# statgen/demuxlet

Measured on AMD Instinct MI355X. Metric: cell-SNP-sample triples/sec (singlet+doublet llk); HBM GB/s vs roofline, higher is better.
Workload: dtype f64

## Files before the change

demuxlet_amd/csrc/dmx_engine.hip:

```cpp
#include <hip/hip_runtime.h>

#include <algorithm>
#include <chrono>
#include <cmath>
#include <mutex>
#include <cstdlib>
#include <cstring>
#include <condition_variable>
#include <deque>
#include <new>
#include <memory>
#include <functional>
#include <thread>
#include <type_traits>
#include <unordered_map>
#include <cxxabi.h>
#include <string>
#include <numeric>
#include <vector>

#include "dmx_internal.hpp"
extern char** environ;
#include "dmx_log.hpp"
#include "dmx_engine_state.hpp"
// ... 2803 lines not shown
  const int64_t np = cell_ok ? pv.cell_pair_off[cell + 1] - p_beg : 0;
  int64_t rd_base = cell_ok ? pv.cell_read_off[cell] : 0;

  const int KB = (V + NK - 1) / NK;
  const int JS = TPC / KB;
  const int jl = tid / KB, kb = tid % KB;
  const int j = (int)blockIdx.y * JS + jl;
  const bool owner = jl < JS && j < V;
  double acc[NK][A];
#pragma unroll
  for (int kk = 0; kk < NK; ++kk) { acc[kk][0] = 0.0; acc[kk][1] = 0.0; }
  bool ok = true;
  const DmxLogPins lk = dmx_log_pins();
  int uj[2] = {0, 0}, uk[2] = {0, 0};
  if constexpr (SYMU) {
#pragma unroll
    for (int su = 0; su < 2; ++su) { const int u = tid + TPC * su; uj[su] = u & (kUV - 1); uk[su] = (uj[su] + 1 + (u >> kUSh)) & (kUV - 1); }
  }
  const int ti1 = tid >> 1, n1 = tid & 1;
  double acc00 = 0.0;
  const int row_len = V * 3;

  for (int64_t tbase = 0; tbase < np; tbase += TP) {
    const int tp = (int)min((int64_t)TP, np - tbase);
    if (tid < TP) {
      const bool v = tid < tp;
      const uint32_t n = v ? load_nrd(pv.pair_nrd, p_beg + tbase + tid, nrd_width) : 0u;
      const uint32_t incl = seg_scan_incl<TP>(n);
      s_cnt[tid] = n;
      s_off[tid] = rd_base + (int64_t)(incl - n);
      s_snp[tid] = v ? (pv.pair_snp ? pv.pair_snp[p_beg + tbase + tid] : (int32_t)(tbase + tid)) : 0;
    }
    DMX_K2_SYNC();
    rd_base = s_off[tp - 1] + (int64_t)s_cnt[tp - 1];
    {
      int r = tid % row_len, ti = tid / row_len;
      const int dr = TPC % row_len, dt = TPC / row_len;
      while (ti < tp) {
        s_g[ti * GS + r] = (g_t)g[(size_t)s_snp[ti] * row_len + r];
        r += dr; ti += dt;
        if (r >= row_len) { r -= row_len; ++ti; }
      }
    }
    if (tid < 2 * TP) {
      const bool on = ti1 < tp;
      const uint32_t cnt = on ? s_cnt[ti1] : 0u;
      const int64_t off = on ? s_off[ti1] : 0;
      const uint32_t rd4 = load_rd4(pv, off, cnt);
      double vf[9];
      const int32_t fi = pfin ? certify_final_index(cnt, rd4) : -1;
      if (!__any(fi < 0)) {
        const double* fp = pfin + (size_t)fi * kCFinStride + (n1 ? 0 : 5);
        const double f0 = fp[0], f1 = fp[1], f2 = fp[2], f3 = n1 ? fp[3] : 0.0, f4 = n1 ? fp[4] : 0.0;
        const double f5[5] = {f0, f1, f2, f3, f4};
#pragma unroll
        for (int l = 0; l < 3; ++l)
#pragma unroll
          for (int m = 0; m < 3; ++m) vf[l * 3 + m] = n1 ? f5[l + m] : f5[l];
      } else if (pseed) {
        double q5[5], wA5[5], wR5[5];
#pragma unroll
        for (int q = 0; q < 5; ++q) {
          const int l = n1 ? (q > 2 ? 2 : q) : min(q, 2), m = n1 ? q - l : 0;
          const double p = 0.5 * l + (m - l) * 0.5 * (n1 ? 0.5 : 0.0);
          wA5[q] = p;
          wR5[q] = 1.0 - p;
        }
        certify_pair_values<5, false>(pv, cnt, off, rd4, s_tab, wA5, wR5, n1, q5, pseed);
#pragma unroll
        for (int l = 0; l < 3; ++l)
#pragma unroll
          for (int m = 0; m < 3; ++m) vf[l * 3 + m] = n1 ? q5[l + m] : q5[l];
      } else {
      double pG[9], wA[9], wR[9];
#pragma unroll
      for (int i = 0; i < 9; ++i) { pG[i] = 1.0; wA[i] = s_w[n1][i]; wR[i] = s_w[n1][9 + i]; }
      for (uint32_t r = 0; __any(r < cnt); ++r) {
        const bool live = r < cnt;
        const uint32_t byte = live ? (r < 4 ? (rd4 >> (8 * r)) & 0xFFu : (uint32_t)pv.reads[off + r]) : 0u;
        const uint32_t bq = byte & 127u;
        const bool alt = (byte >> 7) != 0;
        const double pR = alt ? s_tab[128 + bq] : s_tab[bq];
        const double pA = alt ? s_tab[bq] : s_tab[128 + bq];
        double mx = 0.0;
        if (live) {
#pragma unroll
          for (int i = 0; i < 9; ++i) {
            pG[i] *= (pR * wR[i] + pA * wA[i]);
            mx = fmax(mx, pG[i]);
          }
        }
        {
          const double o = shfl_xor1(mx);
          mx = fmax(mx, o);
        }
        if (live) {
          if (cnt <= kSafeReads) {
            const double y = rcp_refined(mx);
#pragma unroll
            for (int i = 0; i < 9; ++i) pG[i] = div_by(pG[i], mx, y);
          } else {
#pragma unroll
            for (int i = 0; i < 9; ++i) pG[i] /= mx;
          }
        }
      }
      double mx = 0.0;
#pragma unroll
      for (int i = 0; i < 9; ++i) {
        pG[i] += 1e-6;
        mx = fmax(mx, pG[i]);
      }
      {
        const double o = shfl_xor1(mx);
        mx = fmax(mx, o);
      }
      {
        const double y = rcp_refined(mx);
#pragma unroll
        for (int i = 0; i < 9; ++i) vf[i] = div_by(pG[i], mx, y);
      }
      }
      if (on) {
        const double* g0 = gp0 + (size_t)s_snp[ti1] * 3;
        const double q0 = g0[0], q1 = g0[1], q2 = g0[2];
        const double qq[3] = {q0, q1, q2};
        double sum = 0.0;
#pragma unroll
        for (int l = 0; l < 3; ++l)
#pragma unroll
          for (int m = 0; m < 3; ++m) {
            const double v = vf[l * 3 + m];
            s_pG[(ti1 * 2 + n1) * 9 + l * 3 + m] = v;
            sum += ((qq[l] * qq[m]) * v);
          }
        ok &= __builtin_amdgcn_class(sum, 0x100);
        s_t00[n1 * T00 + ti1] = dmx_log2_fast(sum, s_log);
      }
    }
    DMX_K2_SYNC();
    if (tid < 2) {
      const double* row = &s_t00[tid * T00];
      if (tp == TP) {
        double2 v[TP / 2];
#pragma unroll
        for (int i = 0; i < TP / 2; ++i) v[i] = *reinterpret_cast<const double2*>(&row[2 * i]);
#pragma unroll
        for (int i = 0; i < TP / 2; ++i) { acc00 += v[i].x; acc00 += v[i].y; }
      } else {
        for (int i = 0; i < tp; ++i) acc00 += row[i];
      }
    }
    if constexpr (SYMU) {
      for (int ti = 0; ti < tp; ++ti) {
        const double* P = &s_pG[ti * 18];
        const double Q[3] = {P[0], P[3], P[6]};
        const double P1[5] = {P[9], P[10], P[11], P[14], P[17]};
        const g_t* gr = &s_g[ti * GS];
#pragma unroll
        for (int su = 0; su < 2; ++su) {
          const int js = uj[su], ks = uk[su];
          const double a[3] = {(double)gr[js * 3], (double)gr[js * 3 + 1], (double)gr[js * 3 + 2]};
          const double b[3] = {(double)gr[ks * 3], (double)gr[ks * 3 + 1], (double)gr[ks * 3 + 2]};
          double E[3][3];
#pragma unroll
          for (int l = 0; l < 3; ++l)
#pragma unroll
            for (int m = 0; m < 3; ++m) E[l][m] = a[l] * b[m];
          {
            double s_jk0 = E[0][0] * Q[0], s_kj0 = E[0][0] * Q[0];
#pragma unroll
            for (int l = 0; l < 3; ++l)
#pragma unroll
              for (int m = 0; m < 3; ++m) {
                if (l == 0 && m == 0) continue;
                s_jk0 += (E[l][m] * Q[l]);
                s_kj0 += (E[m][l] * Q[l]);
              }
            acc[2 * su][0] += dmx_log2_fast_pinned(s_jk0, s_log, lk);
            acc[2 * su + 1][0] += dmx_log2_fast_pinned(s_kj0, s_log, lk);
          }
          {
#pragma unroll
            for (int l = 0; l < 3; ++l)
#pragma unroll
              for (int m = 0; m < 3; ++m) E[l][m] = E[l][m] * P1[l + m];
            double s_jk1 = E[0][0], s_kj1 = E[0][0];
#pragma unroll
            for (int l = 0; l < 3; ++l)
#pragma unroll
              for (int m = 0; m < 3; ++m) {
                if (l == 0 && m == 0) continue;
                s_jk1 += E[l][m];
                s_kj1 += E[m][l];
              }
            acc[2 * su][1] += dmx_log2_fast_pinned(s_jk1, s_log, lk);
            acc[2 * su + 1][1] += dmx_log2_fast_pinned(s_kj1, s_log, lk);
          }
        }
      }
    } else
    if (owner) {
      for (int ti = 0; ti < tp; ++ti) {
        const double* P = &s_pG[ti * 18];
        double P0[9], P1[9];
#pragma unroll
        for (int i = 0; i < 9; ++i) { P0[i] = P[i]; P1[i] = P[9 + i]; }
        const g_t* gr = &s_g[ti * GS];
        const double a0 = (double)gr[j * 3], a1 = (double)gr[j * 3 + 1], a2 = (double)gr[j * 3 + 2];
        const double aj[3] = {a0, a1, a2};
#pragma unroll
        for (int kk = 0; kk < NK; ++kk) {
          const int k = min(kb * NK + kk, V - 1);
          const double b0 = (double)gr[k * 3], b1 = (double)gr[k * 3 + 1], b2 = (double)gr[k * 3 + 2];
          const double bk[3] = {b0, b1, b2};
          double s0 = (aj[0] * bk[0]) * P0[0], s1 = (aj[0] * bk[0]) * P1[0];
#pragma unroll
          for (int l = 0; l < 3; ++l)
#pragma unroll
            for (int m = 0; m < 3; ++m) {
              if (l == 0 && m == 0) continue;
              const double gp = aj[l] * bk[m];
              s0 += (gp * P0[l * 3 + m]);
              s1 += (gp * P1[l * 3 + m]);
            }
          if (CHK) ok &= __builtin_amdgcn_class(s0, 0x100) && __builtin_amdgcn_class(s1, 0x100);
          acc[kk][0] += dmx_log2_fast_pinned(s0, s_log, lk);
          acc[kk][1] += dmx_log2_fast_pinned(s1, s_log, lk);
        }
      }
    }
    DMX_K2_SYNC();
  }
  if (cell_ok) {
    if constexpr (SYMU) {
#pragma unroll
      for (int su = 0; su < 2; ++su) {
        const int u = tid + TPC * su, d = 1 + (u >> kUSh);
        if (d < kUV / 2 || (d == kUV / 2 && uj[su] < kUV / 2)) {
          double* o = grid + (((size_t)cell * V + uj[su]) * V + uk[su]) * A;
          o[0] = acc[2 * su][0]; o[1] = acc[2 * su][1];
          double* o2 = grid + (((size_t)cell * V + uk[su]) * V + uj[su]) * A;
          o2[0] = acc[2 * su + 1][0]; o2[1] = acc[2 * su + 1][1];
        }
      }
    } else
    if (owner) {
#pragma unroll
      for (int kk = 0; kk < NK; ++kk) {
        const int k = kb * NK + kk;
        if (k < V) {
          double* o = grid + (((size_t)cell * V + j) * V + k) * A;
          o[0] = acc[kk][0]; o[1] = acc[kk][1];
        }
      }
    }
    if (tid < 2 && blockIdx.y == 0) l00[(size_t)cell * A + tid] = acc00;
    if (!ok) flag_cell(flagged, cell);
  }
#undef DMX_K2_SYNC
}
template <int TPC, int NK, int MINW = 1, bool GD = false, bool CHK = true, int TP = 32>
__global__ __launch_bounds__(kThreads, (MINW == 1 && TPC == 64) ? 3 : MINW) void k_doublet_a2(PileupView pv, int nrd_width, const float* __restrict__ g,
                                                         const double* __restrict__ gp0, const double* __restrict__ tabs,
                                                         const double* __restrict__ alpha,
                                                         const int32_t* __restrict__ sched, int32_t V, int32_t GS,
                                                         double* __restrict__ grid, double* __restrict__ l00,
                                                         uint8_t* __restrict__ flagged, const double* __restrict__ pfin, const double* __restrict__ pseed) {
  a2_body<TPC, NK, MINW, GD, CHK, TP, false>(pv, nrd_width, g, gp0, tabs, alpha, sched, V, GS, grid, l00, flagged, pfin, pseed);
}
template <int MINW>
__global__ __launch_bounds__(kThreads, MINW) void k_doublet_a2u(PileupView pv, int nrd_width, const float* __restrict__ g,
                                                          const double* __restrict__ gp0, const double* __restrict__ tabs,
                                                          const double* __restrict__ alpha,
                                                          const int32_t* __restrict__ sched, int32_t V, int32_t GS,
                                                          double* __restrict__ grid, double* __restrict__ l00,
                                                          uint8_t* __restrict__ flagged, const double* __restrict__ pfin, const double* __restrict__ pseed) {
  a2_body<256, 4, MINW, true, false, 32, true>(pv, nrd_width, g, gp0, tabs, alpha, sched, V, GS, grid, l00, flagged, pfin, pseed);
}
__global__ __launch_bounds__(kThreads, 3) void k_doublet_a2u16(PileupView pv, int nrd_width, const float* __restrict__ g,
                                                          const double* __restrict__ gp0, const double* __restrict__ tabs,
                                                          const double* __restrict__ alpha,
                                                          const int32_t* __restrict__ sched, int32_t V, int32_t GS,
                                                          double* __restrict__ grid, double* __restrict__ l00,
                                                          uint8_t* __restrict__ flagged, const double* __restrict__ pfin, const double* __restrict__ pseed) {
  a2_body<64, 4, 1, false, false, 32, true>(pv, nrd_width, g, gp0, tabs, alpha, sched, V, GS, grid, l00, flagged, pfin, pseed);
}

template <int TPC, int NK>
__global__ __launch_bounds__(kThreads, 3) void k_doublet_a2f(PileupView pv, int nrd_width, const float* __restrict__ g,
                                                         const double* __restrict__ gp0, const double* __restrict__ tabs,
                                                         const double* __restrict__ alpha,
                                                         const int32_t* __restrict__ sched, int32_t V, int32_t GS,
                                                         double* __restrict__ grid, double* __restrict__ l00,
                                                         uint8_t* __restrict__ flagged) {
  constexpr int A = 2, TP = 32;
  constexpr int CPW = kThreads / TPC;
  constexpr int T00 = TP + 2;
#define DMX_K2_SYNC() do { if (TPC == 64) { DMX_WAVE_LDS_ORDER(); } else { __syncthreads(); } } while (0)
  extern __shared__ __attribute__((aligned(16))) unsigned char s_raw[];
  __shared__ double s_tab[kTab2];
  const double* s_log = s_tab + kLut2;
  const int t = threadIdx.x;
  stage_k2_tables(s_tab, tabs, t, kThreads);
  __syncthreads();

  const int cw = t / TPC, tid = t % TPC;
  constexpr bool SHARE = TPC > 64;
  constexpr int SUB = 8;
  const int VU = V;
  const size_t cell_bytes = (size_t)TP * 18 * 8 + (size_t)TP * GS * 4 + 2 * T00 * 8 + TP * (4 + 4 + 8) + (SHARE ? (size_t)SUB * 2 * VU * 32 : 0);
  unsigned char* base = s_raw + (size_t)cw * cell_bytes;
  double* s_pG = (double*)base;
  float* s_g = (float*)(base + (size_t)TP * 18 * 8);
  double* s_t00 = (double*)((unsigned char*)s_g + (size_t)TP * GS * 4);
  int64_t* s_off = (int64_t*)(s_t00 + 2 * T00);
  int32_t* s_snp = (int32_t*)(s_off + TP);
  uint32_t* s_cnt = (uint32_t*)(s_snp + TP);
  double* s_u = (double*)(s_cnt + TP);

  const int slot = blockIdx.x * CPW + cw;
  if (TPC == 64 && slot >= pv.B) return;
  const bool cell_ok = slot < pv.B;
  const int32_t cell = cell_ok ? sched[slot] : 0;
  const int64_t p_beg = cell_ok ? pv.cell_pair_off[cell] : 0;
  const int64_t np = cell_ok ? pv.cell_pair_off[cell + 1] - p_beg : 0;
  int64_t rd_base = cell_ok ? pv.cell_read_off[cell] : 0;

  const int KB = (V + NK - 1) / NK;
  const int JS = TPC / KB;
  const int jl = tid / KB, kb = tid % KB;
  const int j = (int)blockIdx.y * JS + jl;
  const bool owner = jl < JS && j < V;
  double acc[NK][A];
#pragma unroll
  for (int kk = 0; kk < NK; ++kk) { acc[kk][0] = 0.0; acc[kk][1] = 0.0; }
  bool ok = true;
  const DmxLogPins lk = dmx_log_pins();
  const int ti1 = tid >> 1, n1 = tid & 1;
  double wA[9], wR[9];
  {
    const double al = alpha[n1];
#pragma unroll
    for (int l = 0; l < 3; ++l)
#pragma unroll
      for (int m = 0; m < 3; ++m) {
        const double p = 0.5 * l + (m - l) * 0.5 * al;
        wA[l * 3 + m] = p;
        wR[l * 3 + m] = 1.0 - p;
      }
  }
  double acc00 = 0.0;
  const int row_len = V * 3;
// ... 782 lines not shown
            for (int l = 0; l < 3; ++l)
#pragma unroll
              for (int m = 0; m < 3; ++m) {
                if (l == 0 && m == 0) continue;
                s_jk0 += (E[l][m] * Q[l]);
                s_kj0 += (E[m][l] * Q[l]);
              }
            acc[i][0] += dmx_log2_fast_pinned(s_jk0, s_log, lk);
            acc[i][2] += dmx_log2_fast_pinned(s_kj0, s_log, lk);
          }
          if (!ROOMY) __builtin_amdgcn_sched_barrier(0);
          {
            const double P[5] = {ROOMY ? Pr[0] : lds_read_f64(&pq[0]), ROOMY ? Pr[1] : lds_read_f64(&pq[1]), ROOMY ? Pr[2] : lds_read_f64(&pq[2]),
                                 ROOMY ? Pr[3] : lds_read_f64(&pq[3]), ROOMY ? Pr[4] : lds_read_f64(&pq[4])};
#pragma unroll
            for (int l = 0; l < 3; ++l)
#pragma unroll
              for (int m = 0; m < 3; ++m) E[l][m] = E[l][m] * P[l + m];
            double s_jk1 = E[0][0], s_kj1 = E[0][0];
#pragma unroll
            for (int l = 0; l < 3; ++l)
#pragma unroll
              for (int m = 0; m < 3; ++m) {
                if (l == 0 && m == 0) continue;
                s_jk1 += E[l][m];
                s_kj1 += E[m][l];
              }
            acc[i][1] += dmx_log2_fast_pinned(s_jk1, s_log, lk);
            acc[i][3] += dmx_log2_fast_pinned(s_kj1, s_log, lk);
          }
          __builtin_amdgcn_sched_barrier(0);
        }
        if (slab == 0) {
          double sd = 0.0;
#pragma unroll
          for (int l = 0; l < 3; ++l)
#pragma unroll
            for (int m = 0; m < 3; ++m) {
              const double v = pq[5 + l + dg[m]];
              const double term = (a[l] * a[m]) * v;
              sd = (l == 0 && m == 0) ? term : sd + term;
            }
          accd += dmx_log2_fast_pinned(sd, s_log, lk);
        }
      }
      DMX_WAVE_LDS_ORDER();
    }
  }
  double* G = grid + (size_t)cell * V * V * A;
#pragma unroll
  for (int i = 0; i < (DIAG_ONLY ? 0 : NU); ++i) {
    const int d = 1 + 2 * (NU * slab + i) + h, k = kk[i];
    if (d < 16 || j < 16) {
      G[((size_t)j * V + k) * A] = acc[i][0]; G[((size_t)j * V + k) * A + 1] = acc[i][1];
      G[((size_t)k * V + j) * A] = acc[i][2]; G[((size_t)k * V + j) * A + 1] = acc[i][3];
    }
  }
  if (slab == 0) {
    G[((size_t)j * V + j) * A + h] = accd;
    if (!DIAG_ONLY && tid < 2) l00[(size_t)cell * A + tid] = acc00;
  }
}

template <int MINW, int VP = 32>
__global__ __launch_bounds__(kThreads, MINW) void k_doublet_diag(PileupView pv, int nrd_width, const float* __restrict__ g,
                                                           const double* __restrict__ tabs, const int32_t* __restrict__ sched,
                                                           double* __restrict__ grid, const double* __restrict__ pfin, const double* __restrict__ pseed) {
  static_assert(VP == 32 || VP == 16, "panel");
  constexpr int V = VP, A = 2, TPC = VP, TP = VP / 2, CPW = kThreads / TPC, row_len = 3 * V, PB = 8, WPC = 64 / TPC;
  __shared__ double s_tab[kTab2];
  __shared__ double s_w[2][10];
  __shared__ __attribute__((aligned(16))) double s_pq_all[CPW][TP][8];
  __shared__ int64_t s_off_all[CPW][TP];
  __shared__ int32_t s_snp_all[CPW][TP];
  __shared__ uint32_t s_cnt_all[CPW][TP];
  const double* s_log = s_tab + kLut2;
  const int t = threadIdx.x;
  stage_k2_tables(s_tab, tabs, t, kThreads);
  if (t < 10) {
    const int n = t / 5, q = t % 5;
    const int l = n ? (q > 2 ? 2 : q) : min(q, 2), m = n ? q - l : 0;
    const double p = 0.5 * l + (m - l) * 0.5 * (n ? 0.5 : 0.0);
    s_w[n][q] = p;
    s_w[n][5 + q] = 1.0 - p;
  }
  __syncthreads();
  const int cw = t / TPC, tid = t % TPC;
  double* s_pq = &s_pq_all[cw][0][0];
  int64_t* s_off = s_off_all[cw]; int32_t* s_snp = s_snp_all[cw]; uint32_t* s_cnt = s_cnt_all[cw];
  const int slot = blockIdx.x * CPW + cw;
  if ((blockIdx.x * CPW + (cw & ~(WPC - 1))) >= pv.B) return;
  const bool cell_ok = slot < pv.B;
  const int32_t cell = cell_ok ? sched[slot] : 0;
  const int64_t p_beg = cell_ok ? pv.cell_pair_off[cell] : 0;
  const int64_t np = cell_ok ? pv.cell_pair_off[cell + 1] - p_beg : 0;
  int64_t rd_base = cell_ok ? pv.cell_read_off[cell] : 0;
  int64_t np_w = np;
#pragma unroll
  for (int d = TPC; d < 64; d <<= 1) { const int64_t o = __shfl_xor(np_w, d); np_w = np_w > o ? np_w : o; }
  const int j = tid;
  double acc0 = 0.0, acc1 = 0.0;
  const DmxLogPins lk = dmx_log_pins();
  const int ti1 = tid >> 1, n1 = tid & 1;
  for (int64_t tbase = 0; tbase < np_w; tbase += TP) {
    const int tp = (int)max((int64_t)0, min((int64_t)TP, np - tbase));
    if (tid < TP) {
      const bool v = tid < tp;
      const uint32_t n = v ? load_nrd(pv.pair_nrd, p_beg + tbase + tid, nrd_width) : 0u;
      const int32_t sn = v ? (pv.pair_snp ? pv.pair_snp[p_beg + tbase + tid] : (int32_t)(tbase + tid)) : 0;
      const uint32_t incl = seg_scan_incl<TP>(n);
      s_cnt[tid] = n;
      s_off[tid] = rd_base + (int64_t)(incl - n);
      s_snp[tid] = sn;
    }
    DMX_WAVE_LDS_ORDER();
    if (tp > 0) rd_base = s_off[tp - 1] + (int64_t)s_cnt[tp - 1];
    {
      const bool on = ti1 < tp;
      const uint32_t cnt = on ? s_cnt[ti1] : 0u;
      const int64_t off = on ? s_off[ti1] : 0;
      const uint32_t rd4 = load_rd4(pv, off, cnt);
      double q[5];
      const int32_t fi = pfin ? certify_final_index(cnt, rd4) : -1;
      if (!__any(fi < 0)) {
        const double* fp = pfin + (size_t)fi * kCFinStride + (n1 ? 0 : 5);
        q[0] = fp[0]; q[1] = fp[1]; q[2] = fp[2];
        q[3] = n1 ? fp[3] : 0.0; q[4] = n1 ? fp[4] : 0.0;
      } else {
        double wA[5], wR[5];
#pragma unroll
        for (int i = 0; i < 5; ++i) { wA[i] = s_w[n1][i]; wR[i] = s_w[n1][5 + i]; }
        certify_pair_values<5, false>(pv, cnt, off, rd4, s_tab, wA, wR, n1, q, pseed);
      }
      if (on) {
        if (n1) {
#pragma unroll
          for (int i = 0; i < 5; ++i) s_pq[ti1 * 8 + i] = q[i];
        } else {
#pragma unroll
          for (int l = 0; l < 3; ++l) s_pq[ti1 * 8 + 5 + l] = q[l];
        }
      }
    }
    DMX_WAVE_LDS_ORDER();
#pragma unroll 1
    for (int sub = 0; sub < TP; sub += PB) {
      if (!__any(sub < tp)) break;
      float ar[PB][3];
#pragma unroll
      for (int pi = 0; pi < PB; ++pi) {
        const float* src = g + (size_t)s_snp[sub + pi] * row_len + j * 3;
        ar[pi][0] = src[0]; ar[pi][1] = src[1]; ar[pi][2] = src[2];
      }
#pragma unroll
      for (int pi = 0; pi < PB; ++pi) {
        if (sub + pi < tp) {
          const double* pq = &s_pq[(sub + pi) * 8];
          const double a[3] = {(double)ar[pi][0], (double)ar[pi][1], (double)ar[pi][2]};
          const double P[5] = {pq[0], pq[1], pq[2], pq[3], pq[4]}, Q[3] = {pq[5], pq[6], pq[7]};
          double s0 = 0.0, s1 = 0.0;
#pragma unroll
          for (int l = 0; l < 3; ++l)
#pragma unroll
            for (int m = 0; m < 3; ++m) {
              const double e = a[l] * a[m];
              const double t0 = e * Q[l], t1 = e * P[l + m];
              s0 = (l == 0 && m == 0) ? t0 : s0 + t0;
              s1 = (l == 0 && m == 0) ? t1 : s1 + t1;
            }
          acc0 += dmx_log2_fast_pinned(s0, s_log, lk);
          acc1 += dmx_log2_fast_pinned(s1, s_log, lk);
        }
      }
    }
    DMX_WAVE_LDS_ORDER();
  }
  if (cell_ok) {
    double* o = grid + (((size_t)cell * V + j) * V + j) * A;
    o[0] = acc0; o[1] = acc1;
  }
}

template <int TPC, int NK, int AP>
__global__ __launch_bounds__(kThreads) void k_doublet_an(PileupView pv, int nrd_width, const float* __restrict__ g,
                                                         const double* __restrict__ gp0, const double* __restrict__ tabs,
                                                         const double* __restrict__ alpha,
                                                         const int32_t* __restrict__ sched, int32_t V, int32_t A, int32_t GS,
                                                         double* __restrict__ grid, double* __restrict__ l00,
                                                         uint8_t* __restrict__ flagged) {
  static_assert(AP == 2 || AP == 4 || AP == 8, "alphas per pair padded to a power of two");
  constexpr int TP = 32;
  constexpr int CPW = kThreads / TPC;
  constexpr int T00 = TP + 2;
#define DMX_K2_SYNC() do { if (TPC == 64) { DMX_WAVE_LDS_ORDER(); } else { __syncthreads(); } } while (0)
  extern __shared__ __attribute__((aligned(16))) unsigned char s_raw[];
  __shared__ double s_tab[kTab2];
  const double* s_log = s_tab + kLut2;
  const int t = threadIdx.x;
  stage_k2_tables(s_tab, tabs, t, kThreads);
  __syncthreads();

  const int cw = t / TPC, tid = t % TPC;
  const size_t cell_bytes = (size_t)TP * AP * 9 * 8 + (size_t)TP * GS * 4 + (size_t)AP * T00 * 8 + TP * (4 + 4 + 8);
  unsigned char* base = s_raw + (size_t)cw * cell_bytes;
  double* s_pG = (double*)base;
  float* s_g = (float*)(base + (size_t)TP * AP * 9 * 8);
  double* s_t00 = (double*)((unsigned char*)s_g + (size_t)TP * GS * 4);
  int64_t* s_off = (int64_t*)(s_t00 + AP * T00);
  int32_t* s_snp = (int32_t*)(s_off + TP);
  uint32_t* s_cnt = (uint32_t*)(s_snp + TP);

  const int slot = blockIdx.x * CPW + cw;
  if (TPC == 64 && slot >= pv.B) return;
  const bool cell_ok = slot < pv.B;
  const int32_t cell = cell_ok ? sched[slot] : 0;
  const int64_t p_beg = cell_ok ? pv.cell_pair_off[cell] : 0;
  const int64_t np = cell_ok ? pv.cell_pair_off[cell + 1] - p_beg : 0;
  int64_t rd_base = cell_ok ? pv.cell_read_off[cell] : 0;

  const int KB = (V + NK - 1) / NK;
  const int JS = TPC / KB;
  const int jl = tid / KB, kb = tid % KB;
  const int j = (int)blockIdx.y * JS + jl;
  const bool owner = jl < JS && j < V;
  double acc[NK][AP];
#pragma unroll
  for (int kk = 0; kk < NK; ++kk)
#pragma unroll
    for (int n = 0; n < AP; ++n) acc[kk][n] = 0.0;
  bool ok = true;
  double acc00 = 0.0;
  const int row_len = V * 3;
  constexpr int P1 = TP * AP;
  constexpr int NPASS = (P1 + TPC - 1) / TPC;
  const int n1 = tid % AP;
  const bool n_ok = n1 < A;
  double wA[9], wR[9];
  {
    const double al = n_ok ? alpha[n1] : 0.0;
#pragma unroll
    for (int l = 0; l < 3; ++l)
#pragma unroll
      for (int m = 0; m < 3; ++m) {
        const double p = 0.5 * l + (m - l) * 0.5 * al;
        wA[l * 3 + m] = p;
        wR[l * 3 + m] = 1.0 - p;
      }
  }

  for (int64_t tbase = 0; tbase < np; tbase += TP) {
    const int tp = (int)min((int64_t)TP, np - tbase);
    if (tid < TP) {
      const bool v = tid < tp;
      const uint32_t n = v ? load_nrd(pv.pair_nrd, p_beg + tbase + tid, nrd_width) : 0u;
      const uint32_t incl = seg_scan_incl<32>(n);
      s_cnt[tid] = n;
      s_off[tid] = rd_base + (int64_t)(incl - n);
      s_snp[tid] = v ? (pv.pair_snp ? pv.pair_snp[p_beg + tbase + tid] : (int32_t)(tbase + tid)) : 0;
    }
    DMX_K2_SYNC();
    rd_base = s_off[tp - 1] + (int64_t)s_cnt[tp - 1];
    {
      int r = tid % row_len, ti = tid / row_len;
      const int dr = TPC % row_len, dt = TPC / row_len;
      while (ti < tp) {
        s_g[ti * GS + r] = g[(size_t)s_snp[ti] * row_len + r];
        r += dr; ti += dt;
        if (r >= row_len) { r -= row_len; ++ti; }
      }
    }
#pragma unroll
    for (int pass = 0; pass < NPASS; ++pass) {
      const int u = tid + pass * TPC;
      if (u >= P1) break;
      const int ti1 = u / AP;
      const bool on = ti1 < tp && n_ok;
      const uint32_t cnt = (ti1 < tp) ? s_cnt[ti1] : 0u;
      const int64_t off = (ti1 < tp) ? s_off[ti1] : 0;
      double pG[9];
#pragma unroll
      for (int i = 0; i < 9; ++i) pG[i] = 1.0;
      for (uint32_t r = 0; __any(r < cnt); ++r) {
        const bool live = r < cnt && n_ok;
        const uint32_t byte = (r < cnt) ? pv.reads[off + r] : 0u;
        const uint32_t bq = byte & 127u;
        const bool alt = (byte >> 7) != 0;
        const double pR = alt ? s_tab[128 + bq] : s_tab[bq];
        const double pA = alt ? s_tab[bq] : s_tab[128 + bq];
        double mx = 0.0;
        if (live) {
#pragma unroll
          for (int i = 0; i < 9; ++i) {
            pG[i] *= (pR * wR[i] + pA * wA[i]);
            mx = fmax(mx, pG[i]);
          }
        }
#pragma unroll
        for (int d = 1; d < AP; d <<= 1) {
          const double o = __shfl_xor(mx, d);
          mx = fmax(mx, o);
        }
        if (live) {
          if (cnt <= kSafeReads) {
            const double y = rcp_refined(mx);
#pragma unroll
            for (int i = 0; i < 9; ++i) pG[i] = div_by(pG[i], mx, y);
          } else {
#pragma unroll
            for (int i = 0; i < 9; ++i) pG[i] /= mx;
          }
        }
      }
      double mx = 0.0;
      if (n_ok) {
#pragma unroll
        for (int i = 0; i < 9; ++i) {
          pG[i] += 1e-6;
          mx = fmax(mx, pG[i]);
        }
      }
#pragma unroll
      for (int d = 1; d < AP; d <<= 1) {
        const double o = __shfl_xor(mx, d);
        mx = fmax(mx, o);
// ... 5178 lines not shown
```

demuxlet_amd/csrc/dmx_log.hpp:

```cpp
#pragma once
#include <stdint.h>
#include <string.h>

#if defined(__HIPCC__)
#include <hip/hip_runtime.h>
#define DMX_HD __host__ __device__ __forceinline__
#else
#include <math.h>
#define DMX_HD static inline
#endif

#include "dmx_log_table.inc"

#define DMX_LOG_TABLE_DOUBLES 256
#define DMX_LOG2_TABLE_DOUBLES 512
#define DMX_LOG32_TABLE_DOUBLES 64

DMX_HD double dmx_log_core_comp(double x, uint32_t hi, uint32_t lo, const double* __restrict__ T) {
  const uint32_t tmp = hi - 0x3FE5F000u;
  const int32_t i = (int32_t)((tmp >> 13) & 127u);
  const int32_t k = (int32_t)tmp >> 20;
  const uint32_t zhi = hi - (tmp & 0xFFF00000u);
  const uint64_t zb = ((uint64_t)zhi << 32) | lo;
  double z;
// ... 46 lines not shown
DMX_HD double dmx_log2_core(uint32_t hi, uint32_t lo, const double* __restrict__ T) {
  const uint32_t tmp = hi - DMX_LOG2_OFF_HI;
  const uint32_t k20 = tmp & 0xFFF00000u;
  const uint32_t zhi = hi - k20;
#if defined(__HIP_DEVICE_COMPILE__)
  const double z = __hiloint2double((int)zhi, (int)lo);
#else
  const uint64_t zb = ((uint64_t)zhi << 32) | lo;
  double z;
  memcpy(&z, &zb, sizeof z);
#endif
  const double* e = reinterpret_cast<const double*>(reinterpret_cast<const char*>(T) + ((tmp >> 8) & 0xFF0u));
  const double invc = e[0], logc = e[1];
  const double r = __builtin_fma(z, invc, -1.0);
  const double kd = (double)(int32_t)k20;
  const double w = __builtin_fma(kd, DMX_LOG_LN2HI * 0x1p-20, logc);
  const double r2 = r * r;
  double t1 = __builtin_fma(r, -0.25, 0x1.5555555555555p-2);
  const double t2 = __builtin_fma(r, -0x1.5555555555555p-3, 0.2);
  t1 = __builtin_fma(r2, t2, t1);
  const double s = __builtin_fma(r, t1, -0.5);
  double p = __builtin_fma(r2, s, r);
  p = __builtin_fma(kd, DMX_LOG_LN2LO * 0x1p-20, p);
  return w + p;
}
DMX_HD double dmx_log2_lite32_core(uint32_t hi, uint32_t lo, const double* __restrict__ T32) {
  const uint32_t tmp = hi - DMX_LOG32_OFF_HI;
  const uint32_t k20 = tmp & 0xFFF00000u;
  const uint32_t zhi = hi - k20;
#if defined(__HIP_DEVICE_COMPILE__)
  const double z = __hiloint2double((int)zhi, (int)lo);
#else
  const uint64_t zb = ((uint64_t)zhi << 32) | lo;
  double z;
  memcpy(&z, &zb, sizeof z);
#endif
  const double* e = reinterpret_cast<const double*>(reinterpret_cast<const char*>(T32) + ((tmp >> 12) & 0xF8u));
  const double rc = e[0], logc = e[32];
  const double r = __builtin_fma(z, rc, -1.0);
  const double kd = (double)(int32_t)k20;
  const double w = __builtin_fma(kd, 0x1.62e42fefa39efp-1 * 0x1p-20, logc);
  double q = __builtin_fma(r, DMX_LOG32_A5, DMX_LOG32_A4);
  q = __builtin_fma(r, q, DMX_LOG32_A3);
  q = __builtin_fma(r, q, DMX_LOG32_A2);
  q = __builtin_fma(r, q, -0.5);
  q = __builtin_fma(r, q, 1.0);
  return __builtin_fma(r, q, w);
}
DMX_HD double dmx_log_core(double x, uint32_t hi, uint32_t lo, const double* __restrict__ T) {
  (void)x;
  return dmx_log_lite_core(hi, lo, T);
}

DMX_HD void dmx_log_dd(uint32_t hiw, uint32_t low, const double* __restrict__ T, const double* __restrict__ T2, double* out_hi, double* out_lo) {
  const uint32_t tmp = hiw - 0x3FE5F000u;
  const int32_t i = (int32_t)((tmp >> 13) & 127u);
  const int32_t k = (int32_t)tmp >> 20;
  const uint32_t zhi = hiw - (tmp & 0xFFF00000u);
#if defined(__HIP_DEVICE_COMPILE__)
  const double z = __hiloint2double((int)zhi, (int)low);
#else
  const uint64_t zb = ((uint64_t)zhi << 32) | low;
  double z;
  memcpy(&z, &zb, sizeof z);
#endif
  const double invc = T[2 * i], logc = T[2 * i + 1], logc_lo = T2[i];
  const double p = z * invc;
  const double pe = __builtin_fma(z, invc, -p);
  const double d = p - 1.0;
  const double rh = d + pe;
  const double rl = (d - rh) + pe;
  const double r2h = rh * rh;
  const double r2l = __builtin_fma(rh, rh, -r2h) + 2.0 * (rh * rl);
  double q = __builtin_fma(rh, -0.1, 0x1.c71c71c71c71cp-4);
  q = __builtin_fma(rh, q, -0.125);
  q = __builtin_fma(rh, q, 0x1.2492492492492p-3);
  q = __builtin_fma(rh, q, -0x1.5555555555555p-3);
  q = __builtin_fma(rh, q, 0.2);
  q = __builtin_fma(rh, q, -0.25);
  q = __builtin_fma(rh, q, 0x1.5555555555555p-2);
  const double t = (rh * r2h) * q;
  const double kd = (double)k;
  const double w = __builtin_fma(kd, DMX_LOG_LN2HI, logc);
  double s = w + rh, bb = s - w;
  const double e1 = (w - (s - bb)) + (rh - bb);
  const double a2 = -0.5 * r2h;
  double s2 = s + a2; bb = s2 - s;
  const double e2 = (s - (s2 - bb)) + (a2 - bb);
  double s3 = s2 + t; bb = s3 - s2;
  const double e3 = (s2 - (s3 - bb)) + (t - bb);
  const double a4 = kd * DMX_LOG_LN2LO;
  double s4 = s3 + a4; bb = s4 - s3;
  const double e4 = (s3 - (s4 - bb)) + (a4 - bb);
  const double tail = ((e1 + e2) + (e3 + e4)) + (((rl - 0.5 * r2l) + logc_lo) + kd * DMX_LOG_LN2LOLO);
  const double h = s4 + tail;
  *out_hi = h;
  *out_lo = (s4 - h) + tail;
}

DMX_HD void dmx_log_bracket(uint32_t hiw, uint32_t low, const double* __restrict__ T, const double* __restrict__ T2, double* t_lo, double* t_hi) {
  double h, l;
  dmx_log_dd(hiw, low, T, T2, &h, &l);
  *t_lo = h; *t_hi = h;
  if (l == 0.0 || h == 0.0) return;
  uint64_t hb;
  memcpy(&hb, &h, sizeof hb);
  const bool away = (l > 0.0) == (h > 0.0);
  const uint64_t nbits = away ? hb + 1 : hb - 1;
  double nb;
  memcpy(&nb, &nbits, sizeof nb);
  const double gap = nb - h;
  const double al = l < 0.0 ? -l : l, ag = gap < 0.0 ? -gap : gap;
  const bool near1 = (hiw - 0x3FEE0000u) < (0x3FF10900u - 0x3FEE0000u);
  if (al > (near1 ? 0.33 : 0.45) * ag) { if (nb < h) *t_lo = nb; else *t_hi = nb; }
}

#if defined(__HIPCC__)
__device__ __forceinline__ bool dmx_log_is_special(double x) { return !__builtin_amdgcn_class(x, 0x100); }
__device__ __forceinline__ double dmx_log_fast(double x, const double* __restrict__ T) {
  return dmx_log_core(x, (uint32_t)__double2hiint(x), (uint32_t)__double2loint(x), T);
}
__device__ __forceinline__ double dmx_log_lite(double x, const double* __restrict__ T) { return dmx_log_fast(x, T); }
struct DmxLogPins { double c13, c15, m14; };
__device__ __forceinline__ DmxLogPins dmx_log_pins() {
  DmxLogPins k{0x1.5555555555555p-2, 0.2, -0.25};
  asm volatile("" : "+v"(k.c13), "+v"(k.c15));
  asm volatile("" : "+s"(k.m14));
  return k;
}
__device__ __forceinline__ double dmx_log_fast_pinned(double x, const double* __restrict__ T, const DmxLogPins& K) {
  const uint32_t hi = (uint32_t)__double2hiint(x), lo = (uint32_t)__double2loint(x);
  const uint32_t tmp = hi - 0x3FE5F000u;
  const uint32_t k20 = tmp & 0xFFF00000u;
  const uint32_t zhi = hi - k20;
  const double z = __hiloint2double((int)zhi, (int)lo);
  const double* e = reinterpret_cast<const double*>(reinterpret_cast<const char*>(T) + ((tmp >> 9) & 0x7F0u));
  const double invc = e[0], logc = e[1];
  const double r = __builtin_fma(z, invc, -1.0);
  const double kd = (double)(int32_t)k20;
  const double w = __builtin_fma(kd, DMX_LOG_LN2HI * 0x1p-20, logc);
  const double r2 = r * r;
  double t1 = __builtin_fma(r, K.m14, K.c13);
  double t2 = __builtin_fma(r, -0x1.5555555555555p-3, K.c15);
  t2 = __builtin_fma(r2, 0x1.2492492492492p-3, t2);
  t1 = __builtin_fma(r2, t2, t1);
  const double s = __builtin_fma(r, t1, -0.5);
  double p = __builtin_fma(r2, s, r);
  p = __builtin_fma(kd, DMX_LOG_LN2LO * 0x1p-20, p);
  return w + p;
}
__device__ __forceinline__ double dmx_log2_fast(double x, const double* __restrict__ T) {
  return dmx_log2_core((uint32_t)__double2hiint(x), (uint32_t)__double2loint(x), T);
}
__device__ __forceinline__ double dmx_log2_fast_pinned(double x, const double* __restrict__ T, const DmxLogPins& K) {
  const uint32_t hi = (uint32_t)__double2hiint(x), lo = (uint32_t)__double2loint(x);
  const uint32_t tmp = hi - DMX_LOG2_OFF_HI;
  const uint32_t k20 = tmp & 0xFFF00000u;
  const uint32_t zhi = hi - k20;
  const double z = __hiloint2double((int)zhi, (int)lo);
  const double* e = reinterpret_cast<const double*>(reinterpret_cast<const char*>(T) + ((tmp >> 8) & 0xFF0u));
  const double invc = e[0], logc = e[1];
  const double r = __builtin_fma(z, invc, -1.0);
  const double kd = (double)(int32_t)k20;
  const double w = __builtin_fma(kd, DMX_LOG_LN2HI * 0x1p-20, logc);
  const double r2 = r * r;
  double t1 = __builtin_fma(r, K.m14, K.c13);
  const double t2 = __builtin_fma(r, -0x1.5555555555555p-3, K.c15);
  t1 = __builtin_fma(r2, t2, t1);
  const double s = __builtin_fma(r, t1, -0.5);
  double p = __builtin_fma(r2, s, r);
  p = __builtin_fma(kd, DMX_LOG_LN2LO * 0x1p-20, p);
  return w + p;
}
__device__ __forceinline__ double dmx_log2_lite(double x, const double* __restrict__ T, const DmxLogPins& K) {
  const uint32_t hi = (uint32_t)__double2hiint(x), lo = (uint32_t)__double2loint(x);
  const uint32_t tmp = hi - DMX_LOG2_OFF_HI;
  const uint32_t k20 = tmp & 0xFFF00000u;
  const uint32_t zhi = hi - k20;
  const double z = __hiloint2double((int)zhi, (int)lo);
  const double* e = reinterpret_cast<const double*>(reinterpret_cast<const char*>(T) + ((tmp >> 8) & 0xFF0u));
  const double invc = e[0], logc = e[1];
  const double r = __builtin_fma(z, invc, -1.0);
  const double kd = (double)(int32_t)k20;
  const double w = __builtin_fma(kd, 0x1.62e42fefa39efp-1 * 0x1p-20, logc);
  double q = __builtin_fma(r, K.m14, K.c13);
  q = __builtin_fma(r, q, -0.5);
  q = __builtin_fma(r, q, 1.0);
  return __builtin_fma(r, q, w);
}
struct DmxLog32Pins { double a5, a4, a3, a2; };
__device__ __forceinline__ DmxLog32Pins dmx_log32_pins() {
  DmxLog32Pins k{DMX_LOG32_A5, DMX_LOG32_A4, DMX_LOG32_A3, DMX_LOG32_A2};
  asm volatile("" : "+v"(k.a4));
  asm volatile("" : "+s"(k.a5), "+s"(k.a3), "+s"(k.a2));
  return k;
}
__device__ __forceinline__ double dmx_log2_lite32(double x, const double* __restrict__ T32, const DmxLog32Pins& K) {
  const uint32_t hi = (uint32_t)__double2hiint(x), lo = (uint32_t)__double2loint(x);
  const uint32_t tmp = hi - DMX_LOG32_OFF_HI;
  const uint32_t k20 = tmp & 0xFFF00000u;
  const uint32_t zhi = hi - k20;
  const double z = __hiloint2double((int)zhi, (int)lo);
  const double* e = reinterpret_cast<const double*>(reinterpret_cast<const char*>(T32) + ((tmp >> 12) & 0xF8u));
  const double rc = e[0], logc = e[32];
  const double r = __builtin_fma(z, rc, -1.0);
  const double kd = (double)(int32_t)k20;
  const double w = __builtin_fma(kd, 0x1.62e42fefa39efp-1 * 0x1p-20, logc);
  double q = __builtin_fma(r, K.a5, K.a4);
  q = __builtin_fma(r, q, K.a3);
  q = __builtin_fma(r, q, K.a2);
  q = __builtin_fma(r, q, -0.5);
  q = __builtin_fma(r, q, 1.0);
  return __builtin_fma(r, q, w);
}
__device__ __forceinline__ double dmx_log(double x, const double* __restrict__ T) {
  const double y = dmx_log_fast(x, T);
  return dmx_log_is_special(x) ? log(x) : y;
}
__device__ __forceinline__ void dmx_log_stage(double* s_tab, const double* __restrict__ g_tab, int tid, int nthreads) {
  for (int i = tid; i < DMX_LOG_TABLE_DOUBLES; i += nthreads) s_tab[i] = g_tab[i];
}
#else
static inline double dmx_log_comp_host_emul(double x) {
  uint64_t b;
  memcpy(&b, &x, sizeof b);
  const uint32_t hi = (uint32_t)(b >> 32), lo = (uint32_t)b;
  if ((hi - 0x00100000u) >= 0x7FE00000u) return log(x);
  return dmx_log_core_comp(x, hi, lo, dmx_log_table_host);
}
static inline double dmx_log2_host_emul(double x) {
  uint64_t b;
  memcpy(&b, &x, sizeof b);
  const uint32_t hi = (uint32_t)(b >> 32), lo = (uint32_t)b;
  if ((hi - 0x00100000u) >= 0x7FE00000u) return log(x);
  return dmx_log2_core(hi, lo, dmx_log2_table_host);
}
static inline double dmx_log2_lite32_host_emul(double x) {
  uint64_t b;
  memcpy(&b, &x, sizeof b);
  const uint32_t hi = (uint32_t)(b >> 32), lo = (uint32_t)b;
  if ((hi - 0x00100000u) >= 0x7FE00000u) return log(x);
  return dmx_log2_lite32_core(hi, lo, dmx_log32_table_host);
}
static inline double dmx_log_host_emul(double x) {
  uint64_t b;
  memcpy(&b, &x, sizeof b);
  const uint32_t hi = (uint32_t)(b >> 32), lo = (uint32_t)b;
  if ((hi - 0x00100000u) >= 0x7FE00000u) return log(x);
  return dmx_log_core(x, hi, lo, dmx_log_table_host);
}
#endif
```

Before: 14.42 billion.

## Software-pipeline log2 table lookups against FMA work in symmetric and diagonal loops

Splits the table-driven log2 into a front half (exponent split plus LDS table load) and a back half (polynomial evaluation). The symmetric-pair loop and the diagonal loop are restructured so each lookup is issued one stage ahead and its polynomial runs after the next stage's sums, with sched_barrier and asm register pins enforcing that order. The goal is to hide LDS load latency behind independent f64 FMAs. In exchange it raises register pressure, adds handling for the final loop iteration, and in the diagonal loop now computes PB entries unconditionally and masks the accumulation.

```diff
diff --git a/demuxlet_amd/csrc/dmx_engine.hip b/demuxlet_amd/csrc/dmx_engine.hip
--- a/demuxlet_amd/csrc/dmx_engine.hip
+++ b/demuxlet_amd/csrc/dmx_engine.hip
@@ -2979,53 +2979,81 @@
       }
     }
     if constexpr (SYMU) {
-      for (int ti = 0; ti < tp; ++ti) {
+      g_t ra[3], rb[3];
+      double Q[3], P1[5], E[3][3];
+      DmxLog2Req pq[2][2];
+      auto req_rows = [&](int ti, int su) {
         const double* P = &s_pG[ti * 18];
-        const double Q[3] = {P[0], P[3], P[6]};
-        const double P1[5] = {P[9], P[10], P[11], P[14], P[17]};
+        Q[0] = P[0]; Q[1] = P[3]; Q[2] = P[6];
         const g_t* gr = &s_g[ti * GS];
-#pragma unroll
-        for (int su = 0; su < 2; ++su) {
-          const int js = uj[su], ks = uk[su];
-          const double a[3] = {(double)gr[js * 3], (double)gr[js * 3 + 1], (double)gr[js * 3 + 2]};
-          const double b[3] = {(double)gr[ks * 3], (double)gr[ks * 3 + 1], (double)gr[ks * 3 + 2]};
-          double E[3][3];
-#pragma unroll
-          for (int l = 0; l < 3; ++l)
-#pragma unroll
-            for (int m = 0; m < 3; ++m) E[l][m] = a[l] * b[m];
-          {
-            double s_jk0 = E[0][0] * Q[0], s_kj0 = E[0][0] * Q[0];
-#pragma unroll
-            for (int l = 0; l < 3; ++l)
-#pragma unroll
-              for (int m = 0; m < 3; ++m) {
-                if (l == 0 && m == 0) continue;
-                s_jk0 += (E[l][m] * Q[l]);
-                s_kj0 += (E[m][l] * Q[l]);
-              }
-            acc[2 * su][0] += dmx_log2_fast_pinned(s_jk0, s_log, lk);
-            acc[2 * su + 1][0] += dmx_log2_fast_pinned(s_kj0, s_log, lk);
+        const int js = uj[su], ks = uk[su];
+        ra[0] = gr[js * 3]; ra[1] = gr[js * 3 + 1]; ra[2] = gr[js * 3 + 2];
+        rb[0] = gr[ks * 3]; rb[1] = gr[ks * 3 + 1]; rb[2] = gr[ks * 3 + 2];
+      };
+      auto sums0 = [&](int ti, int par) {
+        const double* P = &s_pG[ti * 18];
+        const double a[3] = {(double)ra[0], (double)ra[1], (double)ra[2]}, b[3] = {(double)rb[0], (double)rb[1], (double)rb[2]};
+#pragma unroll
+        for (int l = 0; l < 3; ++l)
+#pragma unroll
+          for (int m = 0; m < 3; ++m) E[l][m] = a[l] * b[m];
+        double s_jk0 = E[0][0] * Q[0], s_kj0 = E[0][0] * Q[0];
+#pragma unroll
+        for (int l = 0; l < 3; ++l)
+#pragma unroll
+          for (int m = 0; m < 3; ++m) {
+            if (l == 0 && m == 0) continue;
+            s_jk0 += (E[l][m] * Q[l]);
+            s_kj0 += (E[m][l] * Q[l]);
           }
-          {
-#pragma unroll
-            for (int l = 0; l < 3; ++l)
-#pragma unroll
-              for (int m = 0; m < 3; ++m) E[l][m] = E[l][m] * P1[l + m];
-            double s_jk1 = E[0][0], s_kj1 = E[0][0];
-#pragma unroll
-            for (int l = 0; l < 3; ++l)
-#pragma unroll
-              for (int m = 0; m < 3; ++m) {
-                if (l == 0 && m == 0) continue;
-                s_jk1 += E[l][m];
-                s_kj1 += E[m][l];
-              }
-            acc[2 * su][1] += dmx_log2_fast_pinned(s_jk1, s_log, lk);
-            acc[2 * su + 1][1] += dmx_log2_fast_pinned(s_kj1, s_log, lk);
+        pq[par][0] = dmx_log2_pinned_front(s_jk0, s_log);
+        pq[par][1] = dmx_log2_pinned_front(s_kj0, s_log);
+        P1[0] = P[9]; P1[1] = P[10]; P1[2] = P[11]; P1[3] = P[14]; P1[4] = P[17];
+      };
+      auto sums1 = [&](int par) {
+#pragma unroll
+        for (int l = 0; l < 3; ++l)
+#pragma unroll
+          for (int m = 0; m < 3; ++m) E[l][m] = E[l][m] * P1[l + m];
+        double s_jk1 = E[0][0], s_kj1 = E[0][0];
+#pragma unroll
+        for (int l = 0; l < 3; ++l)
+#pragma unroll
+          for (int m = 0; m < 3; ++m) {
+            if (l == 0 && m == 0) continue;
+            s_jk1 += E[l][m];
+            s_kj1 += E[m][l];
           }
-        }
-      }
+        pq[par][0] = dmx_log2_pinned_front(s_jk1, s_log);
+        pq[par][1] = dmx_log2_pinned_front(s_kj1, s_log);
+      };
+#define DMX_A2U_BACK(su, n, par, NEXT) do { \
+        asm volatile("" ::: "memory");                \
+        __builtin_amdgcn_sched_barrier(0);            \
+        asm volatile("" : "+v"(pq[par][0].invc), "+v"(pq[par][1].invc)); \
+        acc[2 * (su)][n] += dmx_log2_pinned_back(pq[par][0], lk);               \
+        acc[2 * (su) + 1][n] += dmx_log2_pinned_back(pq[par][1], lk); \
+        __builtin_amdgcn_sched_barrier(0); \
+        if ((NEXT) == 0) asm volatile("" : "+v"(ra[0]), "+v"(rb[0]));           \
+        if ((NEXT) == 1) asm volatile("" : "+v"(P1[0])); } while (0)
+      auto pair = [&](int ti, bool last) __attribute__((always_inline)) {
+        sums1(1);
+        req_rows(ti, 1);
+        DMX_A2U_BACK(0, 0, 0, 0);
+        sums0(ti, 0);
+        DMX_A2U_BACK(0, 1, 1, 1);
+        sums1(1);
+        if (!last) req_rows(ti + 1, 0);
+        DMX_A2U_BACK(1, 0, 0, last ? 2 : 0);
+        if (!last) sums0(ti + 1, 0);
+        DMX_A2U_BACK(1, 1, 1, last ? 2 : 1);
+      };
+      const int tpu = __builtin_amdgcn_readfirstlane(tp);
+      req_rows(0, 0);
+      sums0(0, 0);
+      for (int ti = 0; ti + 1 < tpu; ++ti) pair(ti, false);
+      pair(tpu - 1, true);
+#undef DMX_A2U_BACK
     } else
     if (owner) {
       for (int ti = 0; ti < tp; ++ti) {
@@ -4114,9 +4142,10 @@
         const float* src = g + (size_t)s_snp[sub + pi] * row_len + j * 3;
         ar[pi][0] = src[0]; ar[pi][1] = src[1]; ar[pi][2] = src[2];
       }
-#pragma unroll
-      for (int pi = 0; pi < PB; ++pi) {
-        if (sub + pi < tp) {
+      DmxLog2Req dq[2][2];
+#pragma unroll
+      for (int pi = 0; pi <= PB; ++pi) {
+        if (pi < PB) {
           const double* pq = &s_pq[(sub + pi) * 8];
           const double a[3] = {(double)ar[pi][0], (double)ar[pi][1], (double)ar[pi][2]};
           const double P[5] = {pq[0], pq[1], pq[2], pq[3], pq[4]}, Q[3] = {pq[5], pq[6], pq[7]};
@@ -4130,8 +4159,20 @@
               s0 = (l == 0 && m == 0) ? t0 : s0 + t0;
               s1 = (l == 0 && m == 0) ? t1 : s1 + t1;
             }
-          acc0 += dmx_log2_fast_pinned(s0, s_log, lk);
-          acc1 += dmx_log2_fast_pinned(s1, s_log, lk);
+          dq[pi & 1][0] = dmx_log2_pinned_front(s0, s_log);
+          dq[pi & 1][1] = dmx_log2_pinned_front(s1, s_log);
+        }
+        if (pi > 0) {
+          const int pv1 = (pi - 1) & 1;
+          const bool live = sub + pi - 1 < tp;
+          asm volatile("" ::: "memory");
+          __builtin_amdgcn_sched_barrier(0);
+          asm volatile("" : "+v"(dq[pv1][0].invc), "+v"(dq[pv1][1].invc));
+          const double t0 = dmx_log2_pinned_back(dq[pv1][0], lk), t1 = dmx_log2_pinned_back(dq[pv1][1], lk);
+          acc0 = live ? acc0 + t0 : acc0;
+          acc1 = live ? acc1 + t1 : acc1;
+          __builtin_amdgcn_sched_barrier(0);
+          if (pi < PB) asm volatile("" : "+v"(ar[pi][0]));
         }
       }
     }
diff --git a/demuxlet_amd/csrc/dmx_log.hpp b/demuxlet_amd/csrc/dmx_log.hpp
--- a/demuxlet_amd/csrc/dmx_log.hpp
+++ b/demuxlet_amd/csrc/dmx_log.hpp
@@ -222,17 +222,20 @@
 __device__ __forceinline__ double dmx_log2_fast(double x, const double* __restrict__ T) {
   return dmx_log2_core((uint32_t)__double2hiint(x), (uint32_t)__double2loint(x), T);
 }
-__device__ __forceinline__ double dmx_log2_fast_pinned(double x, const double* __restrict__ T, const DmxLogPins& K) {
+struct DmxLog2Req { double z; int32_t k20; double invc, logc; };
+__device__ __forceinline__ DmxLog2Req dmx_log2_pinned_front(double x, const double* __restrict__ T) {
   const uint32_t hi = (uint32_t)__double2hiint(x), lo = (uint32_t)__double2loint(x);
   const uint32_t tmp = hi - DMX_LOG2_OFF_HI;
   const uint32_t k20 = tmp & 0xFFF00000u;
   const uint32_t zhi = hi - k20;
   const double z = __hiloint2double((int)zhi, (int)lo);
   const double* e = reinterpret_cast<const double*>(reinterpret_cast<const char*>(T) + ((tmp >> 8) & 0xFF0u));
-  const double invc = e[0], logc = e[1];
-  const double r = __builtin_fma(z, invc, -1.0);
-  const double kd = (double)(int32_t)k20;
-  const double w = __builtin_fma(kd, DMX_LOG_LN2HI * 0x1p-20, logc);
+  return DmxLog2Req{z, (int32_t)k20, e[0], e[1]};
+}
+__device__ __forceinline__ double dmx_log2_pinned_back(const DmxLog2Req& q, const DmxLogPins& K) {
+  const double r = __builtin_fma(q.z, q.invc, -1.0);
+  const double kd = (double)q.k20;
+  const double w = __builtin_fma(kd, DMX_LOG_LN2HI * 0x1p-20, q.logc);
   const double r2 = r * r;
   double t1 = __builtin_fma(r, K.m14, K.c13);
   const double t2 = __builtin_fma(r, -0x1.5555555555555p-3, K.c15);
@@ -241,6 +244,9 @@
   double p = __builtin_fma(r2, s, r);
   p = __builtin_fma(kd, DMX_LOG_LN2LO * 0x1p-20, p);
   return w + p;
+}
+__device__ __forceinline__ double dmx_log2_fast_pinned(double x, const double* __restrict__ T, const DmxLogPins& K) {
+  return dmx_log2_pinned_back(dmx_log2_pinned_front(x, T), K);
 }
 __device__ __forceinline__ double dmx_log2_lite(double x, const double* __restrict__ T, const DmxLogPins& K) {
   const uint32_t hi = (uint32_t)__double2hiint(x), lo = (uint32_t)__double2loint(x);
```

Result: no change. 14.55 billion (median of 6 runs) (+0.9%).
